# iammadab/zk

Hardware: AMD Instinct MI355X
Metric: field-ops/sec (MLE fold, 2^24 evals, BN254 Fr) + sumcheck prover wall-clock (higher is better)
Workload: dtype u256 (8 x u32 Montgomery limbs, integer)

## Files before the change

### zk_amd/csrc/gkr.hip

```cpp
#include <hip/hip_runtime.h>

#include <new>
#include <utility>
#include <vector>

#include "../../include/zk_amd.h"
#include "host_core.hpp"
#include "env.hpp"
#include "gkr_kernels.cuh"
#include "prover_state.hpp"


struct GkrLayer {
    uint32_t log_out, log_in;
    uint64_t n_gates, n_in;
    uint8_t *d_op;
    uint32_t *d_left, *d_right;
    uint32_t *d_lptr, *d_rptr;
    uint2 *d_lent, *d_rent;
    uint32_t *d_lheavy, *d_rheavy;
    uint32_t n_lheavy, n_rheavy;
    uint32_t *d_lptr_light, *d_rptr_light;
    uint2 *d_lent_light, *d_rent_light;
    uint8_t digest[112];
// ... 8 lines not shown
extern "C" int32_t zk_circuit_create(zk_ctx *c, zk_circuit **out) {
    if (!c || !out) return ZK_ERR_BAD_ARG;
    zk_circuit *z = new (std::nothrow) zk_circuit();
    if (!z) return ZK_ERR_ALLOC;
    z->ctx = c;
    *out = z;
    return ZK_OK;
}
extern "C" int32_t zk_circuit_free(zk_circuit *z) {
    if (!z) return ZK_OK;
    (void)use_device(z->ctx);
    delete z;
    return ZK_OK;
}
extern "C" int32_t zk_circuit_depth(const zk_circuit *z, uint64_t *out) {
    if (!z || !out) return ZK_ERR_BAD_ARG;
    *out = z->layers.size();
    return ZK_OK;
}
extern "C" int32_t zk_circuit_layer_dims(const zk_circuit *z, uint64_t layer, uint64_t *log_out, uint64_t *log_in) {
    if (!z || layer >= z->layers.size() || !log_out || !log_in) return ZK_ERR_BAD_ARG;
    *log_out = z->layers[layer].log_out;
    *log_in = z->layers[layer].log_in;
    return ZK_OK;
}
extern "C" int32_t zk_circuit_proof_elems(const zk_circuit *z, uint64_t *out) {
    if (!z || !out) return ZK_ERR_BAD_ARG;
    uint64_t n = 0;
    for (const auto &L : z->layers) n += 6ull * L.log_in + 2;
    *out = n;
    return ZK_OK;
}

static int32_t gkr_tree_reduce(zk_ctx *c, uint64_t *buf_a, uint64_t *buf_b, uint64_t n, uint64_t **root) {
    uint64_t *cur = buf_a, *nxt = buf_b;
    while (n > 1) {
        const uint64_t n_out = (n + 3) / 4;
        if (n_out <= 4096) k_tree_level_wave<<<(uint32_t)n_out, 64, 0, c->stream>>>(cur, n, nxt);
        else k_tree_level<<<grid_for(n_out), kBlock, 0, c->stream>>>(cur, n, n_out, nxt);
        HIPCHK(hipGetLastError());
        std::swap(cur, nxt);
        n = n_out;
    }
    *root = cur;
    return ZK_OK;
}
static int32_t gkr_table_digest_dev(zk_ctx *c, const zk_mle *t, uint64_t *d_out) {
    const uint64_t n = 1ull << t->n_vars, n_leaves = (n + 3) / 4;
    PoolScope ps(c);
    uint64_t *a = nullptr, *b = nullptr, *root = nullptr;
    ZKCHK(ps.get((size_t)n_leaves * 32, &a));
    ZKCHK(ps.get((size_t)((n_leaves + 3) / 4) * 32, &b));
    k_tree_leaves_table<<<grid_for(n_leaves), kBlock, 0, c->stream>>>(t->d, n, n_leaves, a, c->fi->P);
    HIPCHK(hipGetLastError());
    ZKCHK(gkr_tree_reduce(c, a, b, n_leaves, &root));
    HIPCHK(hipMemcpyAsync(d_out, root, 32, hipMemcpyDeviceToDevice, c->stream));
    return ZK_OK;
}
static int32_t gkr_bytes_digest(zk_ctx *c, const void *d_data, uint64_t nbytes, uint8_t out[32]) {
    const uint64_t n_leaves = nbytes ? (nbytes + 127) / 128 : 1;
    PoolScope ps(c);
    uint64_t *a = nullptr, *b = nullptr, *root = nullptr;
    ZKCHK(ps.get((size_t)n_leaves * 32, &a));
    ZKCHK(ps.get((size_t)((n_leaves + 3) / 4) * 32, &b));
    k_tree_leaves_bytes<<<grid_for(n_leaves), kBlock, 0, c->stream>>>((const uint8_t *)d_data, nbytes, n_leaves, a);
    HIPCHK(hipGetLastError());
    ZKCHK(gkr_tree_reduce(c, a, b, n_leaves, &root));
    HIPCHK(hipMemcpyAsync(out, root, 32, hipMemcpyDeviceToHost, c->stream));
    HIPCHK(hipStreamSynchronize(c->stream));
    return ZK_OK;
}
static void put_u64le(uint8_t *p, uint64_t v) {
    for (int i = 0; i < 8; ++i) p[i] = (uint8_t)(v >> (8 * i));
}
static void gkr_circuit_digest(const zk_circuit *z, uint8_t out[32]) {
    Sponge h;
    h.init();
    for (const auto &L : z->layers) h.update(L.digest, sizeof L.digest);
    h.finalize_reset(out);
}

template <typename T>
static int32_t gkr_upload(GkrLayer &L, T **dst, const T *src, size_t count) {
    if (L.n_blocks == (int)(sizeof L.blocks / sizeof L.blocks[0])) return ZK_ERR_ALLOC;
    RawBlock b;
    HIPCHK(hipMalloc(b.put(), (count ? count : 1) * sizeof(T)));
    if (count) HIPCHK(hipMemcpy(b.get(), src, count * sizeof(T), hipMemcpyHostToDevice));
    *dst = static_cast<T *>(b.get());
    L.blocks[L.n_blocks++] = std::move(b);
    return ZK_OK;
}
static int32_t gkr_upload_light(GkrLayer &L, const std::vector<uint32_t> &ptr, const std::vector<uint2> &ent, const std::vector<uint32_t> &heavy,
                                uint32_t *d_ptr, uint2 *d_ent, uint32_t **d_ptr_light, uint2 **d_ent_light) {
    if (heavy.empty()) {
        *d_ptr_light = d_ptr;
        *d_ent_light = d_ent;
        return ZK_OK;
    }
    const size_t rows = ptr.size() - 1;
    std::vector<uint32_t> lp(rows + 1, 0);
    std::vector<uint2> le;
// ... 72 lines not shown
    uint64_t *d_hi = nullptr, *d_lo = nullptr;
    ZKCHK(ps.get((size_t)32 << hi_bits, &d_hi));
    ZKCHK(ps.get((size_t)32 << lo_bits, &d_lo));
    {
        if (m <= 30) {
            const size_t lds = ((size_t)2 << ((lo_bits + 1) / 2)) * 32 + (size_t)2 * lo_bits * 32 + 64;
            k_eq_halves<<<2, kBlock, lds, c->stream>>>(d_point, (uint32_t)m, scale, d_hi, d_lo, P, d_scale);
        } else {
            k_eq_direct<<<grid_for(1ull << hi_bits), kBlock, 0, c->stream>>>(d_point, (uint32_t)hi_bits, scale, d_hi, P, d_scale);
            k_eq_direct<<<grid_for(1ull << lo_bits), kBlock, 0, c->stream>>>(d_point + 4 * hi_bits, (uint32_t)lo_bits, fe_one(P), d_lo, P);
        }
        if (accumulate)
            k_eq_outer<true><<<grid_for(1ull << m), kBlock, 0, c->stream>>>(d_hi, d_lo, (uint32_t)lo_bits, 1ull << m, d_out, P);
        else
            k_eq_outer<false><<<grid_for(1ull << m), kBlock, 0, c->stream>>>(d_hi, d_lo, (uint32_t)lo_bits, 1ull << m, d_out, P);
        HIPCHK(hipGetLastError());
    }
    return ZK_OK;
}
int32_t zk::eq_table_dev(zk_ctx *c, const uint64_t *d_point, uint64_t m, uint64_t *d_out) {
    return gkr_eq_table_dev(c, d_point, m, fe_one(c->fi->P), false, d_out);
}
static int32_t gkr_upload_point(zk_ctx *c, const uint64_t *point, uint64_t m, uint64_t *d_point) {
    if (m == 0) return ZK_OK;
    HIPCHK(hipMemcpyAsync(d_point, point, (size_t)m * 32, hipMemcpyHostToDevice, c->stream));
    HIPCHK(hipStreamSynchronize(c->stream));
    return ZK_OK;
}
struct EqHalves {
    PoolBlock buf;
    EqFactor f = {};
    void reset() { buf.reset(); }
};
static int32_t gkr_eq_halves(zk_ctx *c, const uint64_t *d_p1, const uint64_t *d_s1, const uint64_t *d_p2, const uint64_t *d_s2, uint64_t m,
                             EqHalves *out) {
    const FieldParams &P = c->fi->P;
    out->reset();
    out->f = {};
    if (m > 30) return ZK_ERR_UNSUPPORTED;
    const uint32_t lo_bits = eq_split_lo_bits(m), hi_bits = (uint32_t)m - lo_bits;
    const size_t hb = (size_t)32 << hi_bits, lb = (size_t)(kEqLoWords * 4) << lo_bits;
    ZKCHK(out->buf.alloc(c, (d_p2 ? 2 : 1) * (hb + lb)));
    uint64_t *hi1 = out->buf.as(), *lo1 = hi1 + hb / 8, *hi2 = d_p2 ? lo1 + lb / 8 : nullptr, *lo2 = d_p2 ? hi2 + hb / 8 : nullptr;
    const uint32_t bh = ((1u << hi_bits) + 1023) / 1024, bl = ((1u << lo_bits) + 1023) / 1024;
    const EqSplitJob j0 = {d_p1, d_s1, hi1, reinterpret_cast<uint32_t *>(lo1)}, j1 = {d_p2, d_s2, hi2, reinterpret_cast<uint32_t *>(lo2)};
    k_eq_split<<<(d_p2 ? 2 : 1) * (bh + bl), kBlock, 0, c->stream>>>(j0, j1, (uint32_t)m, lo_bits, bh, bl, P);
    HIPCHK(hipGetLastError());
    out->f = {hi1, hi2, reinterpret_cast<const uint32_t *>(lo1), reinterpret_cast<const uint32_t *>(lo2), lo_bits};
    return ZK_OK;
}
static int32_t gkr_eq_table(zk_ctx *c, const uint64_t *point, uint64_t m, const Fe *scale, bool accumulate, uint64_t *d_out) {
    PoolBlock d_point;
    ZKCHK(d_point.alloc(c, (size_t)(m ? m : 1) * 32));
    ZKCHK(gkr_upload_point(c, point, m, d_point.as()));
    return gkr_eq_table_dev(c, d_point.as(), m, scale ? *scale : fe_one(c->fi->P), accumulate, d_out);
}
extern "C" int32_t zk_eq_table(zk_ctx *c, const uint64_t *point, uint64_t n_vars, zk_mle **out) {
    if (!c || !out || (!point && n_vars)) return ZK_ERR_BAD_ARG;
    if (n_vars > kMaxVars) return ZK_ERR_UNSUPPORTED;
    ZKCHK(use_device(c));
    MleHolder t;
    ZKCHK(mle_alloc(c, n_vars, t.put()));
    ZKCHK(gkr_eq_table(c, point, n_vars, nullptr, false, t->d));
    *out = t.release();
    return ZK_OK;
}

static int32_t gkr_check_input(const zk_circuit *z, const zk_mle *input) {
    if (!z || !input) return ZK_ERR_BAD_ARG;
    if (z->layers.empty()) return ZK_ERR_BAD_ARG;
    if (input->ctx != z->ctx) return ZK_ERR_CONTEXT_MISMATCH;
    if (input->n_vars != z->layers.back().log_in) return ZK_ERR_ARITY_MISMATCH;
    return use_device(z->ctx);
}
struct GkrValues {
    std::vector<MleHolder> own;
    std::vector<zk_mle *> vals;
};
static int32_t gkr_forward(const zk_circuit *z, const zk_mle *input, GkrValues &v) {
    zk_ctx *c = z->ctx;
    const size_t d = z->layers.size();
    v.own.resize(d);
    v.vals.assign(d + 1, nullptr);
    v.vals[d] = const_cast<zk_mle *>(input);
    for (size_t i = d; i-- > 0;) {
        const GkrLayer &L = z->layers[i];
        ZKCHK(mle_alloc(c, L.log_out, v.own[i].put()));
        v.vals[i] = v.own[i].get();
        k_gkr_forward<<<grid_for(L.n_gates), kBlock, 0, c->stream>>>(L.d_op, L.d_left, L.d_right, v.vals[i + 1]->d, L.n_gates, v.vals[i]->d, c->fi->P);
        HIPCHK(hipGetLastError());
    }
    return ZK_OK;
}
extern "C" int32_t zk_gkr_evaluate(const zk_circuit *z, const zk_mle *input, zk_mle **out_outputs) {
    if (!out_outputs) return ZK_ERR_BAD_ARG;
    ZKCHK(gkr_check_input(z, input));
    GkrValues v;
    ZKCHK(gkr_forward(z, input, v));
    *out_outputs = v.own[0].release();
    return ZK_OK;
}

struct GkrClaim {
    std::vector<uint64_t> g1, g2;
    Fe alpha, beta, c;
    bool two;
};
static int32_t gkr_start(const zk_circuit *z, const zk_mle *input, const zk_mle *outputs, Sponge &sp, const uint8_t seed[32], GkrClaim &cl) {
    zk_ctx *c = z->ctx;
    const FieldParams &P = c->fi->P;
    const uint64_t log_out0 = z->layers[0].log_out;
    uint8_t cd[32], io[64];
    gkr_circuit_digest(z, cd);
    {
        PoolBlock d_dig;
        ZKCHK(d_dig.alloc(c, 64));
        ZKCHK(gkr_table_digest_dev(c, input, d_dig.as()));
        ZKCHK(gkr_table_digest_dev(c, outputs, d_dig.as() + 4));
        HIPCHK(hipMemcpyAsync(c->h_pinned, d_dig.p, 64, hipMemcpyDeviceToHost, c->stream));
        HIPCHK(hipStreamSynchronize(c->stream));
    }
    memcpy(io, c->h_pinned, 64);
    sp.init();
    sp.update(seed, 32);
    sp.update(cd, 32);
    sp.update(io, 64);
    cl.g1.assign(4 * log_out0, 0);
    for (uint64_t i = 0; i < log_out0; ++i) fe_to_u64limbs(squeeze_field_element(sp, P), cl.g1.data() + 4 * i);
    cl.g2.clear();
    cl.alpha = fe_one(P);
    cl.beta = fe_zero();
    cl.two = false;
    return ZK_OK;
}
static void gkr_next_claim(Sponge &sp, const FieldParams &P, const uint64_t *layer_proof, uint64_t log_in, const uint64_t *u,
                           const uint64_t *v, GkrClaim &cl) {
    cl.alpha = squeeze_field_element(sp, P);
    cl.beta = squeeze_field_element(sp, P);
    cl.two = true;
    cl.g1.assign(u, u + 4 * log_in);
    cl.g2.assign(v, v + 4 * log_in);
    const Fe wu = fe_from_u64limbs(layer_proof + 4 * (6 * log_in)), wv = fe_from_u64limbs(layer_proof + 4 * (6 * log_in + 1));
    cl.c = fe_add(fe_mul(cl.alpha, wu, P), fe_mul(cl.beta, wv, P), P);
}

extern "C" int32_t zk_gkr_prove(const zk_circuit *z, const zk_mle *input, const uint8_t seed[32], zk_mle **out_outputs,
                                uint64_t *out_proof) {
    if (!seed || !out_outputs || !out_proof) return ZK_ERR_BAD_ARG;
    ZKCHK(gkr_check_input(z, input));
    zk_ctx *c = z->ctx;
    const FieldParams &P = c->fi->P;
    const size_t d = z->layers.size();
    GkrValues v;
    PoolScope ps(c);
    DrainOnExit drain(c);
    ZKCHK(gkr_forward(z, input, v));
    const std::vector<zk_mle *> &vals = v.vals;
    uint64_t proof_elems = 0;
    (void)zk_circuit_proof_elems(z, &proof_elems);
    Sponge sp;
    GkrClaim cl;
    ZKCHK(gkr_start(z, input, vals[0], sp, seed, cl));
    constexpr size_t kPointBytes = 64 * 32;
    uint64_t *d_pt[4] = {nullptr, nullptr, nullptr, nullptr}, *d_fin = nullptr, *d_sc = nullptr, *d_proof = nullptr;
    WordSponge *d_sponge = nullptr;
    for (int i = 0; i < 4; ++i) ZKCHK(ps.get(kPointBytes, &d_pt[i]));
    ZKCHK(ps.get(kMaxFactors * 32, &d_fin));
    ZKCHK(ps.get(kGkrScalars * 32, &d_sc));
    ZKCHK(ps.get(sizeof(WordSponge), &d_sponge));
    ZKCHK(ps.get((size_t)proof_elems * 32, &d_proof));
    uint64_t *d_epart = nullptr;
    ZKCHK(ps.get(kEpartBlockBytes, &d_epart));
    uint64_t *d_g1 = d_pt[0], *d_g2 = d_pt[1], *d_u = d_pt[2], *d_v = d_pt[3];
    ZKCHK(gkr_upload_point(c, cl.g1.data(), z->layers[0].log_out, d_g1));
    ZKCHK(sponge_to_device(c, sp, d_sponge, d_epart));
    ZKCHK(evaluate_device(c, vals[0], cl.g1.data(), d_sc + 4 * kGkrScClaim));
    k_gkr_chain_start<<<1, 64, 0, c->stream>>>(d_sponge, d_sc, P);
    HIPCHK(hipGetLastError());
    bool two = false;
    uint64_t *proof = d_proof;
    for (size_t i = 0; i < d; ++i) {
        const GkrLayer &L = z->layers[i];
        const uint64_t s = L.log_in;
        MleHolder H, B, H2, C2;
        ZKCHK(mle_alloc(c, s, H.put()));
        ZKCHK(mle_alloc(c, s, B.put()));
        ZKCHK(mle_alloc(c, s, H2.put()));
        ZKCHK(mle_alloc(c, s, C2.put()));
        EqHalves hE, hU;
        ZKCHK(gkr_eq_halves(c, d_g1, two ? d_sc + 4 * kGkrScAlpha : nullptr, two ? d_g2 : nullptr, two ? d_sc + 4 * kGkrScBeta : nullptr, L.log_out, &hE));
        k_gkr_phase<1><<<gkr_phase_grid(L.n_in), kBlock, 0, c->stream>>>(L.d_lptr_light, L.d_lent_light, hE.f, vals[i + 1]->d, EqFactor{}, nullptr, L.n_in,
                                                                         H->d, B->d, P);
        if (L.n_lheavy) k_gkr_phase1_heavy<<<L.n_lheavy, kBlock, 0, c->stream>>>(L.d_lheavy, L.d_lptr, L.d_lent, hE.f, vals[i + 1]->d, H->d, B->d, P);
        HIPCHK(hipGetLastError());
        TermSpec ts = {2, {2, 1, 0, 0}};
        zk_mle *f1[3] = {vals[i + 1], H.get(), B.get()};
        const DeviceChain ch1 = {d_sponge, proof, d_u, d_fin, d_epart};
        ZKCHK(prove_core(c, f1, 3, ts, 2, nullptr, 0, 0, nullptr, nullptr, nullptr, nullptr, nullptr, nullptr, &ch1));
        k_gkr_chain_mid<<<1, 64, 0, c->stream>>>(d_sponge, d_fin, proof + 4 * (6 * s), d_sc, P);
        HIPCHK(hipGetLastError());
        ZKCHK(gkr_eq_halves(c, d_u, nullptr, d_u, d_fin, s, &hU));
        k_gkr_phase<2><<<gkr_phase_grid(L.n_in), kBlock, 0, c->stream>>>(L.d_rptr_light, L.d_rent_light, hE.f, nullptr, hU.f, d_fin, L.n_in, H2->d, C2->d, P);
        if (L.n_rheavy) k_gkr_phase2_heavy<<<L.n_rheavy, kBlock, 0, c->stream>>>(L.d_rheavy, L.d_rptr, L.d_rent, hE.f, hU.f, d_fin, H2->d, C2->d, P);
        HIPCHK(hipGetLastError());
        hE.reset();
        hU.reset();
        zk_mle *f2[3] = {vals[i + 1], H2.get(), C2.get()};
        const DeviceChain ch2 = {d_sponge, proof + 4 * (3 * s), d_v, d_fin, d_epart};
        ZKCHK(prove_core(c, f2, 3, ts, 2, nullptr, 0, 0, nullptr, nullptr, nullptr, nullptr, nullptr, nullptr, &ch2));
        k_gkr_chain_end<<<1, 64, 0, c->stream>>>(d_sponge, d_fin, proof + 4 * (6 * s), proof + 4 * (6 * s + 1), d_sc, P);
        HIPCHK(hipGetLastError());
        proof += 4 * (6 * s + 2);
        std::swap(d_g1, d_u);
        std::swap(d_g2, d_v);
        two = true;
    }
    HIPCHK(hipMemcpyAsync(out_proof, d_proof, (size_t)proof_elems * 32, hipMemcpyDeviceToHost, c->stream));
    ZKCHK(drain.wait());
    *out_outputs = v.own[0].release();
    return ZK_OK;
}

struct GkrLayerCheck {
    Fe sub2, wu, wv;
};
extern "C" int32_t zk_gkr_verify(const zk_circuit *z, const zk_mle *input, const zk_mle *outputs, const uint8_t seed[32],
                                 const uint64_t *proof_in) {
    if (!seed || !outputs || !proof_in) return ZK_ERR_BAD_ARG;
    ZKCHK(gkr_check_input(z, input));
    zk_ctx *c = z->ctx;
    if (outputs->ctx != c) return ZK_ERR_CONTEXT_MISMATCH;
    if (outputs->n_vars != z->layers[0].log_out) return ZK_ERR_ARITY_MISMATCH;
    const FieldParams &P = c->fi->P;
    const size_t d = z->layers.size();
// ... 121 lines not shown
```

### zk_amd/csrc/gkr_kernels.cuh

```cuda
#pragma once
#include "common.cuh"
#include "transcript.cuh"

namespace zk {

__global__ __launch_bounds__(kBlock) void k_eq_direct(const uint64_t *__restrict__ point, uint32_t nv, Fe scale,
                                                      uint64_t *__restrict__ out, FieldParams P, const uint64_t *__restrict__ d_scale = nullptr) {
    if (d_scale) scale = fe_load(d_scale, 0);
    const uint64_t n = 1ull << nv, stride = (uint64_t)gridDim.x * kBlock;
    Fe one;
#pragma unroll
    for (int i = 0; i < 8; ++i) one.v[i] = P.r1[i];
    for (uint64_t j = (uint64_t)blockIdx.x * kBlock + threadIdx.x; j < n; j += stride) {
        Fe acc = scale;
        for (uint32_t w = 0; w < nv; ++w) {
            const Fe g = fe_load(point, w);
            const bool bit = (j >> (nv - 1 - w)) & 1;
            acc = fe_mul(acc, bit ? g : fe_sub(one, g, P), P);
        }
        fe_store(out, j, acc);
    }
}
template <bool ACCUMULATE>
__global__ __launch_bounds__(kBlock) void k_eq_outer(const uint64_t *__restrict__ hi, const uint64_t *__restrict__ lo,
// ... 52 lines not shown
        const uint32_t j = in_a ? e : e - na, cnt = in_a ? a : b, off = in_a ? 0 : a;
        Fe acc = (in_a && is_hi) ? scale : one;
        for (uint32_t w = 0; w < cnt; ++w) acc = fe_mul(acc, fe_load(pt, 2 * (off + w) + ((j >> (cnt - 1 - w)) & 1)), P);
        fe_store(in_a ? qa : qb, j, acc);
    }
    __syncthreads();
    uint64_t *dst = is_hi ? d_hi : d_lo;
    for (uint32_t i = threadIdx.x; i < (1u << nv); i += kBlock) fe_store(dst, i, fe_mul(fe_load(qa, i >> b), fe_load(qb, i & (nb - 1)), P));
}

struct EqFactor {
    const uint64_t *hi, *hi2;
    const uint32_t *lo, *lo2;
    uint32_t lo_bits;
};
ZK_D Fe eq_factor_at(const EqFactor &f, uint32_t i, const FieldParams &P) {
    const uint32_t h = i >> f.lo_bits, l = i & ((1u << f.lo_bits) - 1);
    const Fe a = fe_load(f.hi, h);
    const Mul29 c = load_eq_lo(f.lo + (size_t)l * kEqLoWords);
    if (!f.hi2) return fe_mul29(a, c, P);
    return fe_dot2_29(a, c, fe_load(f.hi2, h), load_eq_lo(f.lo2 + (size_t)l * kEqLoWords), P);
}

ZK_D Fe eq_u_at(const EqFactor &f, uint32_t i, bool scaled, const FieldParams &P) {
    const uint32_t h = i >> f.lo_bits, l = i & ((1u << f.lo_bits) - 1);
    return fe_mul29(fe_load(scaled ? f.hi2 : f.hi, h), load_eq_lo(f.lo + (size_t)l * kEqLoWords), P);
}
struct EqSplitJob {
    const uint64_t *point, *scale;
    uint64_t *hi;
    uint32_t *lo;
};
static inline uint32_t eq_split_lo_bits(uint64_t m) { return (uint32_t)(m <= 7 ? m : (m > 23 ? m - 16 : 7)); }
__global__ __launch_bounds__(kBlock) void k_eq_split(EqSplitJob j0, EqSplitJob j1, uint32_t m, uint32_t lo_bits, uint32_t bh, uint32_t bl,
                                                     FieldParams P) {
    __shared__ uint64_t qa[256 * 4], qb[256 * 4], pt[2 * 16 * 4];
    const uint32_t per = bh + bl, slot = blockIdx.x % per;
    const EqSplitJob job = blockIdx.x / per ? j1 : j0;
    const bool is_hi = slot < bh;
    const uint32_t slice = is_hi ? slot : slot - bh;
    const uint32_t nv = is_hi ? m - lo_bits : lo_bits, first = is_hi ? 0 : m - lo_bits;
    const uint32_t a = nv / 2, b = nv - a, na = 1u << a, nb = 1u << b;
    Fe one;
#pragma unroll
    for (int i = 0; i < 8; ++i) one.v[i] = P.r1[i];
    if (threadIdx.x < nv) {
        const Fe g = fe_load(job.point, first + threadIdx.x);
        fe_store(pt, 2 * threadIdx.x, fe_sub(one, g, P));
        fe_store(pt, 2 * threadIdx.x + 1, g);
    }
    __syncthreads();
    const Fe scale = (is_hi && job.scale) ? fe_load(job.scale, 0) : one;
    for (uint32_t e = threadIdx.x; e < na + nb; e += kBlock) {
        const bool in_a = e < na;
        const uint32_t j = in_a ? e : e - na, cnt = in_a ? a : b, off = in_a ? 0 : a;
        Fe acc = in_a ? scale : one;
        for (uint32_t w = 0; w < cnt; ++w) acc = fe_mul(acc, fe_load(pt, 2 * (off + w) + ((j >> (cnt - 1 - w)) & 1)), P);
        fe_store(in_a ? qa : qb, j, acc);
    }
    __syncthreads();
    const uint32_t end = (slice + 1) * 1024 < (1u << nv) ? (slice + 1) * 1024 : (1u << nv);
    for (uint32_t i = slice * 1024 + threadIdx.x; i < end; i += kBlock) {
        const Fe v = fe_mul(fe_load(qa, i >> b), fe_load(qb, i & (nb - 1)), P);
        if (is_hi) fe_store(job.hi, i, v);
        else store_eq_lo(job.lo + (size_t)i * kEqLoWords, mul29_prepare(v, P));
    }
}

__global__ __launch_bounds__(kBlock) void k_gkr_forward(const uint8_t *__restrict__ op, const uint32_t *__restrict__ left,
                                                        const uint32_t *__restrict__ right, const uint64_t *__restrict__ W,
                                                        uint64_t n_gates, uint64_t *__restrict__ out, FieldParams P) {
    const uint64_t stride = (uint64_t)gridDim.x * kBlock;
    for (uint64_t z = (uint64_t)blockIdx.x * kBlock + threadIdx.x; z < n_gates; z += stride) {
        const Fe a = fe_load(W, left[z]), b = fe_load(W, right[z]);
        fe_store(out, z, op[z] ? fe_mul(a, b, P) : fe_add(a, b, P));
    }
}

constexpr uint32_t kGkrHeavyRow = 256;
ZK_D void gkr_block_sum2(Fe (&sum)[2], const FieldParams &P) {
    __shared__ uint32_t red2[kBlock / 64][2][8];
    const int lane = threadIdx.x & 63, wave = threadIdx.x >> 6;
#pragma unroll
    for (int t = 0; t < 2; ++t) {
        sum[t] = fe_wave_sum(sum[t], P);
        if (lane == 0) {
#pragma unroll
            for (int i = 0; i < 8; ++i) red2[wave][t][i] = sum[t].v[i];
        }
    }
    __syncthreads();
    if (threadIdx.x == 0) {
#pragma unroll
        for (int t = 0; t < 2; ++t) {
            Fe acc = fe_zero();
            for (int w = 0; w < kBlock / 64; ++w) {
                Fe o;
#pragma unroll
                for (int i = 0; i < 8; ++i) o.v[i] = red2[w][t][i];
                acc = fe_add(acc, o, P);
            }
            sum[t] = acc;
        }
    }
}
__global__ __launch_bounds__(kBlock) void k_gkr_phase1_heavy(const uint32_t *__restrict__ heavy, const uint32_t *__restrict__ lptr,
                                                             const uint2 *__restrict__ lent, EqFactor E,
                                                             const uint64_t *__restrict__ W, uint64_t *__restrict__ H,
                                                             uint64_t *__restrict__ B1, FieldParams P) {
// ... 129 lines not shown
    const uint64_t stride = (uint64_t)gridDim.x * kBlock, first = (uint64_t)blockIdx.x * kBlock + threadIdx.x;
    if (first >= n) return;
    Fe cur = scale, b = base;
    for (uint64_t e = first; e; e >>= 1) {
        if (e & 1) cur = fe_mul(cur, b, P);
        b = fe_mul(b, b, P);
    }
    for (uint64_t j = first; j < n; j += stride) {
        fe_store(t, j, fe_mul(fe_load(t, j), cur, P));
        cur = fe_mul(cur, step, P);
    }
}
__global__ __launch_bounds__(kBlock) void k_dft_across(const uint64_t *__restrict__ in, uint64_t *__restrict__ out, uint32_t W,
                                                       uint64_t L, const uint64_t *__restrict__ pw, FieldParams P) {
    const uint64_t stride = (uint64_t)gridDim.x * kBlock;
    for (uint64_t j = (uint64_t)blockIdx.x * kBlock + threadIdx.x; j < L; j += stride) {
        for (uint32_t k = 0; k < W; ++k) {
            Fe acc = fe_load(in, j);
            for (uint32_t r = 1; r < W; ++r) acc = fe_add(acc, fe_mul(fe_load(in, (uint64_t)r * L + j), fe_load(pw, (r * k) & (W - 1)), P), P);
            fe_store(out, (uint64_t)k * L + j, acc);
        }
    }
}

constexpr int kGkrScClaim = 0, kGkrScAlpha = 1, kGkrScBeta = 2, kGkrScSum2 = 3, kGkrScalars = 4;
__global__ __launch_bounds__(64) void k_gkr_chain_start(WordSponge *__restrict__ gsp, const uint64_t *__restrict__ sc, FieldParams P) {
    __shared__ Fe buf[2];
    const LaneKeccak L = lane_keccak_init();
    LaneSponge sp = lane_sponge_load(gsp, L);
    if (L.lane == 0) buf[0] = fe_load(sc, kGkrScClaim);
    lane_absorb_elems(sp, L, buf, 1, P);
    lane_sponge_store(gsp, sp, L);
}
__global__ __launch_bounds__(64) void k_gkr_chain_mid(WordSponge *__restrict__ gsp, const uint64_t *__restrict__ fin, uint64_t *__restrict__ proof_wu,
                                                       uint64_t *__restrict__ sc, FieldParams P) {
    __shared__ Fe buf[2];
    const LaneKeccak L = lane_keccak_init();
    LaneSponge sp = lane_sponge_load(gsp, L);
    if (L.lane == 0) {
        const Fe wu = fe_load(fin, 0), hu = fe_load(fin, 1), bu = fe_load(fin, 2);
        const Fe s2 = fe_add(fe_mul(wu, hu, P), bu, P);
        buf[0] = wu;
        buf[1] = s2;
        fe_store(proof_wu, 0, wu);
        fe_store(sc, kGkrScSum2, s2);
    }
    lane_absorb_elems(sp, L, buf, 2, P);
    lane_sponge_store(gsp, sp, L);
}
__global__ __launch_bounds__(64) void k_gkr_chain_end(WordSponge *__restrict__ gsp, const uint64_t *__restrict__ fin, const uint64_t *__restrict__ proof_wu,
                                                       uint64_t *__restrict__ proof_wv, uint64_t *__restrict__ sc, FieldParams P) {
    __shared__ Fe buf[2];
    const LaneKeccak L = lane_keccak_init();
    LaneSponge sp = lane_sponge_load(gsp, L);
    const Fe wu = fe_load(proof_wu, 0), wv = fe_load(fin, 0);
    if (L.lane == 0) {
        buf[0] = wv;
        fe_store(proof_wv, 0, wv);
    }
    lane_absorb_elems(sp, L, buf, 1, P);
    Mul29 t29;
    const Fe alpha = lane_squeeze(sp, L, P, t29), beta = lane_squeeze(sp, L, P, t29);
    const Fe claim = fe_add(fe_mul(alpha, wu, P), fe_mul(beta, wv, P), P);
    if (L.lane == 0) {
        buf[1] = claim;
        fe_store(sc, kGkrScAlpha, alpha);
        fe_store(sc, kGkrScBeta, beta);
        fe_store(sc, kGkrScClaim, claim);
    }
    lane_absorb_elems(sp, L, buf + 1, 1, P);
    lane_sponge_store(gsp, sp, L);
}

ZK_D void tree_keccak_finish(uint64_t (&s)[25], uint32_t len_bytes, uint64_t *__restrict__ out) {
    s[len_bytes >> 3] ^= 0x01ull << (8 * (len_bytes & 7));
    s[16] ^= 0x8000000000000000ull;
    keccak_f1600(s);
#pragma unroll
    for (int i = 0; i < 4; ++i) out[i] = s[i];
}
__global__ __launch_bounds__(kBlock) void k_tree_leaves_table(const uint64_t *__restrict__ table, uint64_t n_elems, uint64_t n_leaves,
                                                              uint64_t *__restrict__ out, FieldParams P) {
    const uint64_t stride = (uint64_t)gridDim.x * kBlock;
    for (uint64_t i = (uint64_t)blockIdx.x * kBlock + threadIdx.x; i < n_leaves; i += stride) {
        uint64_t s[25];
#pragma unroll
        for (int k = 0; k < 25; ++k) s[k] = 0;
        uint32_t len = 0;
#pragma unroll
        for (int e = 0; e < 4; ++e) {
            if (4 * i + e < n_elems) {
                const Fe c = fe_to_canonical(fe_load(table, 4 * i + e), P);
#pragma unroll
                for (int w = 0; w < 4; ++w)
                    s[4 * e + w] = WordSponge::bswap64((uint64_t)c.v[2 * (3 - w)] | ((uint64_t)c.v[2 * (3 - w) + 1] << 32));
                len += 32;
            }
        }
        tree_keccak_finish(s, len, out + 4 * i);
    }
}
__global__ __launch_bounds__(kBlock) void k_tree_leaves_bytes(const uint8_t *__restrict__ data, uint64_t nbytes, uint64_t n_leaves,
                                                              uint64_t *__restrict__ out) {
    const uint64_t stride = (uint64_t)gridDim.x * kBlock;
    for (uint64_t i = (uint64_t)blockIdx.x * kBlock + threadIdx.x; i < n_leaves; i += stride) {
        uint64_t s[25];
#pragma unroll
        for (int k = 0; k < 25; ++k) s[k] = 0;
        const uint64_t base = 128 * i;
        const uint32_t len = (uint32_t)(nbytes - base < 128 ? nbytes - base : 128);
#pragma unroll
        for (int w = 0; w < 16; ++w) {
            uint64_t x = 0;
            for (int b = 0; b < 8; ++b)
                if ((uint32_t)(8 * w + b) < len) x |= (uint64_t)data[base + 8 * w + b] << (8 * b);
            s[w] = x;
        }
        tree_keccak_finish(s, len, out + 4 * i);
    }
}
__global__ __launch_bounds__(kBlock) void k_tree_level(const uint64_t *__restrict__ in, uint64_t n_in, uint64_t n_out, uint64_t *__restrict__ out) {
    const uint64_t stride = (uint64_t)gridDim.x * kBlock;
    for (uint64_t j = (uint64_t)blockIdx.x * kBlock + threadIdx.x; j < n_out; j += stride) {
        uint64_t s[25];
#pragma unroll
        for (int k = 0; k < 25; ++k) s[k] = 0;
        uint32_t len = 0;
#pragma unroll
        for (int c = 0; c < 4; ++c) {
            if (4 * j + c < n_in) {
#pragma unroll
                for (int w = 0; w < 4; ++w) s[4 * c + w] = in[4 * (4 * j + c) + w];
                len += 32;
            }
        }
        tree_keccak_finish(s, len, out + 4 * j);
    }
}
__global__ __launch_bounds__(64) void k_tree_level_wave(const uint64_t *__restrict__ in, uint64_t n_in, uint64_t *__restrict__ out) {
    const uint64_t j = blockIdx.x;
    const LaneKeccak L = lane_keccak_init();
    const uint64_t rem = n_in - 4 * j;
    const uint32_t nwords = 4 * (uint32_t)(rem < 4 ? rem : 4);
    uint64_t a = 0;
    if (L.index >= 0 && (uint32_t)L.index < nwords) a = in[16 * j + (uint32_t)L.index];
    if ((uint32_t)L.index == nwords) a ^= 0x01ull;
    if (L.index == 16) a ^= 0x8000000000000000ull;
    a = lane_keccak_f1600(a, L);
    if (L.index >= 0 && L.index < 4) out[4 * j + (uint32_t)L.index] = a;
}

}
```

Before: 195.1 billion.

## Fuse Merkle tree levels in LDS and piggyback hashing on GKR kernels

Replaces the per-level Keccak Merkle reduction (one launch per 4:1 level) with a block-local kernel that computes leaves and several levels inside shared memory. Two independent tree chains (input and output digests) now run in one 2D launch. The input-table digest is spread across the GKR forward-pass launches as extra blocks, and the chain-mid sponge step is merged into the eq-split launch. The aim is to cut kernel launches and global round trips, at the cost of more shared-memory use and more complex kernels.

```diff
diff --git a/zk_amd/csrc/gkr.hip b/zk_amd/csrc/gkr.hip
--- a/zk_amd/csrc/gkr.hip
+++ b/zk_amd/csrc/gkr.hip
@@ -64,41 +64,69 @@
     return ZK_OK;
 }
 
-static int32_t gkr_tree_reduce(zk_ctx *c, uint64_t *buf_a, uint64_t *buf_b, uint64_t n, uint64_t **root) {
-    uint64_t *cur = buf_a, *nxt = buf_b;
-    while (n > 1) {
-        const uint64_t n_out = (n + 3) / 4;
-        if (n_out <= 4096) k_tree_level_wave<<<(uint32_t)n_out, 64, 0, c->stream>>>(cur, n, nxt);
-        else k_tree_level<<<grid_for(n_out), kBlock, 0, c->stream>>>(cur, n, n_out, nxt);
+struct TreeChain {
+    TreeJob job = {};
+    uint64_t *buf[2] = {nullptr, nullptr}, *dst = nullptr;
+    int flip = 0;
+    bool done = true;
+};
+static int32_t tree_chain_begin(PoolScope &ps, TreeChain &t, uint32_t kind, const void *src, uint64_t n_src, uint64_t n_leaves, uint64_t *dst,
+                                uint32_t first_unit = kTreeUnit) {
+    t = TreeChain();
+    t.job = {src, n_src, n_leaves, nullptr, kind};
+    t.dst = dst;
+    t.done = false;
+    const uint64_t n1 = (n_leaves + first_unit - 1) / first_unit, n2 = (n1 + kTreeUnit - 1) / kTreeUnit;
+    if (n1 > 1) ZKCHK(ps.get((size_t)n1 * 32, &t.buf[0]));
+    if (n2 > 1) ZKCHK(ps.get((size_t)n2 * 32, &t.buf[1]));
+    return ZK_OK;
+}
+static uint64_t tree_chain_stage(TreeChain &t, uint32_t unit) {
+    const uint64_t units = (t.job.n + unit - 1) / unit;
+    t.job.out = units == 1 ? t.dst : t.buf[t.flip];
+    return units;
+}
+static void tree_chain_advance(TreeChain &t, uint64_t units) {
+    if (units == 1) {
+        t.done = true;
+        return;
+    }
+    t.job = {t.job.out, 0, units, nullptr, kTreeDigests};
+    t.flip ^= 1;
+}
+static int32_t tree_chains_run(zk_ctx *c, TreeChain *a, TreeChain *b) {
+    TreeChain *all[2] = {a, b};
+    for (;;) {
+        TreeChain *who[2];
+        TreeJob j[2] = {};
+        uint64_t units[2] = {0, 0};
+        uint32_t nj = 0;
+        for (TreeChain *t : all) {
+            if (!t || t->done) continue;
+            units[nj] = tree_chain_stage(*t, kTreeUnit);
+            j[nj] = t->job;
+            who[nj++] = t;
+        }
+        if (!nj) return ZK_OK;
+        const uint64_t gx = units[0] > units[1] ? units[0] : units[1];
+        if (gx > 0x7FFFFFFFull) return ZK_ERR_UNSUPPORTED;
+        k_tree_stage<<<dim3((uint32_t)gx, nj), kBlock, 0, c->stream>>>(j[0], j[1], c->fi->P);
         HIPCHK(hipGetLastError());
-        std::swap(cur, nxt);
-        n = n_out;
-    }
-    *root = cur;
-    return ZK_OK;
-}
-static int32_t gkr_table_digest_dev(zk_ctx *c, const zk_mle *t, uint64_t *d_out) {
-    const uint64_t n = 1ull << t->n_vars, n_leaves = (n + 3) / 4;
+        for (uint32_t i = 0; i < nj; ++i) tree_chain_advance(*who[i], units[i]);
+    }
+}
+static int32_t tree_chain_begin_table(PoolScope &ps, TreeChain &t, const zk_mle *tab, uint64_t *dst, uint32_t first_unit = kTreeUnit) {
+    const uint64_t n = 1ull << tab->n_vars;
+    return tree_chain_begin(ps, t, kTreeTable, tab->d, n, (n + 3) / 4, dst, first_unit);
+}
+static int32_t gkr_bytes_digest(zk_ctx *c, const void *d_data, uint64_t nbytes, uint8_t out[32]) {
     PoolScope ps(c);
-    uint64_t *a = nullptr, *b = nullptr, *root = nullptr;
-    ZKCHK(ps.get((size_t)n_leaves * 32, &a));
-    ZKCHK(ps.get((size_t)((n_leaves + 3) / 4) * 32, &b));
-    k_tree_leaves_table<<<grid_for(n_leaves), kBlock, 0, c->stream>>>(t->d, n, n_leaves, a, c->fi->P);
-    HIPCHK(hipGetLastError());
-    ZKCHK(gkr_tree_reduce(c, a, b, n_leaves, &root));
-    HIPCHK(hipMemcpyAsync(d_out, root, 32, hipMemcpyDeviceToDevice, c->stream));
-    return ZK_OK;
-}
-static int32_t gkr_bytes_digest(zk_ctx *c, const void *d_data, uint64_t nbytes, uint8_t out[32]) {
-    const uint64_t n_leaves = nbytes ? (nbytes + 127) / 128 : 1;
-    PoolScope ps(c);
-    uint64_t *a = nullptr, *b = nullptr, *root = nullptr;
-    ZKCHK(ps.get((size_t)n_leaves * 32, &a));
-    ZKCHK(ps.get((size_t)((n_leaves + 3) / 4) * 32, &b));
-    k_tree_leaves_bytes<<<grid_for(n_leaves), kBlock, 0, c->stream>>>((const uint8_t *)d_data, nbytes, n_leaves, a);
-    HIPCHK(hipGetLastError());
-    ZKCHK(gkr_tree_reduce(c, a, b, n_leaves, &root));
-    HIPCHK(hipMemcpyAsync(out, root, 32, hipMemcpyDeviceToHost, c->stream));
+    uint64_t *d_root = nullptr;
+    ZKCHK(ps.get(32, &d_root));
+    TreeChain t;
+    ZKCHK(tree_chain_begin(ps, t, kTreeBytes, d_data, nbytes, nbytes ? (nbytes + 127) / 128 : 1, d_root));
+    ZKCHK(tree_chains_run(c, &t, nullptr));
+    HIPCHK(hipMemcpyAsync(out, d_root, 32, hipMemcpyDeviceToHost, c->stream));
     HIPCHK(hipStreamSynchronize(c->stream));
     return ZK_OK;
 }
@@ -237,8 +265,13 @@
     EqFactor f = {};
     void reset() { buf.reset(); }
 };
+struct GkrMidStep {
+    WordSponge *sponge;
+    const uint64_t *fin;
+    uint64_t *proof_wu, *sc;
+};
 static int32_t gkr_eq_halves(zk_ctx *c, const uint64_t *d_p1, const uint64_t *d_s1, const uint64_t *d_p2, const uint64_t *d_s2, uint64_t m,
-                             EqHalves *out) {
+                             EqHalves *out, const GkrMidStep *mid = nullptr) {
     const FieldParams &P = c->fi->P;
     out->reset();
     out->f = {};
@@ -249,7 +282,9 @@
     uint64_t *hi1 = out->buf.as(), *lo1 = hi1 + hb / 8, *hi2 = d_p2 ? lo1 + lb / 8 : nullptr, *lo2 = d_p2 ? hi2 + hb / 8 : nullptr;
     const uint32_t bh = ((1u << hi_bits) + 1023) / 1024, bl = ((1u << lo_bits) + 1023) / 1024;
     const EqSplitJob j0 = {d_p1, d_s1, hi1, reinterpret_cast<uint32_t *>(lo1)}, j1 = {d_p2, d_s2, hi2, reinterpret_cast<uint32_t *>(lo2)};
-    k_eq_split<<<(d_p2 ? 2 : 1) * (bh + bl), kBlock, 0, c->stream>>>(j0, j1, (uint32_t)m, lo_bits, bh, bl, P);
+    const uint32_t g = (d_p2 ? 2 : 1) * (bh + bl);
+    if (mid) k_gkr_chain_mid_eq<<<1 + g, kBlock, 0, c->stream>>>(mid->sponge, mid->fin, mid->proof_wu, mid->sc, j0, j1, (uint32_t)m, lo_bits, bh, bl, P);
+    else k_eq_split<<<g, kBlock, 0, c->stream>>>(j0, j1, (uint32_t)m, lo_bits, bh, bl, P);
     HIPCHK(hipGetLastError());
     out->f = {hi1, hi2, reinterpret_cast<const uint32_t *>(lo1), reinterpret_cast<const uint32_t *>(lo2), lo_bits};
     return ZK_OK;
@@ -282,19 +317,27 @@
     std::vector<MleHolder> own;
     std::vector<zk_mle *> vals;
 };
-static int32_t gkr_forward(const zk_circuit *z, const zk_mle *input, GkrValues &v) {
+static int32_t gkr_forward(const zk_circuit *z, const zk_mle *input, GkrValues &v, TreeChain *rider = nullptr) {
     zk_ctx *c = z->ctx;
     const size_t d = z->layers.size();
     v.own.resize(d);
     v.vals.assign(d + 1, nullptr);
     v.vals[d] = const_cast<zk_mle *>(input);
-    for (size_t i = d; i-- > 0;) {
+    const uint64_t units = rider ? tree_chain_stage(*rider, kTreeRiderUnit) : 0;
+    for (size_t i = d, k = 0; i-- > 0; ++k) {
         const GkrLayer &L = z->layers[i];
         ZKCHK(mle_alloc(c, L.log_out, v.own[i].put()));
         v.vals[i] = v.own[i].get();
-        k_gkr_forward<<<grid_for(L.n_gates), kBlock, 0, c->stream>>>(L.d_op, L.d_left, L.d_right, v.vals[i + 1]->d, L.n_gates, v.vals[i]->d, c->fi->P);
+        TreeRider r = {};
+        if (rider) {
+            const uint64_t first = units * k / d;
+            r = {rider->job, (uint32_t)first, (uint32_t)(units * (k + 1) / d - first)};
+        }
+        k_gkr_forward<<<r.n_units + grid_for(L.n_gates), kBlock, 0, c->stream>>>(L.d_op, L.d_left, L.d_right, v.vals[i + 1]->d, L.n_gates, v.vals[i]->d,
+                                                                               c->fi->P, r);
         HIPCHK(hipGetLastError());
     }
+    if (rider) tree_chain_advance(*rider, units);
     return ZK_OK;
 }
 extern "C" int32_t zk_gkr_evaluate(const zk_circuit *z, const zk_mle *input, zk_mle **out_outputs) {
@@ -311,18 +354,24 @@
     Fe alpha, beta, c;
     bool two;
 };
-static int32_t gkr_start(const zk_circuit *z, const zk_mle *input, const zk_mle *outputs, Sponge &sp, const uint8_t seed[32], GkrClaim &cl) {
+static int32_t gkr_start(const zk_circuit *z, const zk_mle *input, const zk_mle *outputs, Sponge &sp, const uint8_t seed[32], GkrClaim &cl,
+                         TreeChain *in_chain = nullptr, uint64_t *d_dig = nullptr) {
     zk_ctx *c = z->ctx;
     const FieldParams &P = c->fi->P;
     const uint64_t log_out0 = z->layers[0].log_out;
     uint8_t cd[32], io[64];
     gkr_circuit_digest(z, cd);
     {
-        PoolBlock d_dig;
-        ZKCHK(d_dig.alloc(c, 64));
-        ZKCHK(gkr_table_digest_dev(c, input, d_dig.as()));
-        ZKCHK(gkr_table_digest_dev(c, outputs, d_dig.as() + 4));
-        HIPCHK(hipMemcpyAsync(c->h_pinned, d_dig.p, 64, hipMemcpyDeviceToHost, c->stream));
+        PoolScope ps(c);
+        TreeChain t_in, t_out;
+        if (!in_chain) {
+            ZKCHK(ps.get(64, &d_dig));
+            ZKCHK(tree_chain_begin_table(ps, t_in, input, d_dig));
+            in_chain = &t_in;
+        }
+        ZKCHK(tree_chain_begin_table(ps, t_out, outputs, d_dig + 4));
+        ZKCHK(tree_chains_run(c, &t_out, in_chain));
+        HIPCHK(hipMemcpyAsync(c->h_pinned, d_dig, 64, hipMemcpyDeviceToHost, c->stream));
         HIPCHK(hipStreamSynchronize(c->stream));
     }
     memcpy(io, c->h_pinned, 64);
@@ -359,13 +408,17 @@
     GkrValues v;
     PoolScope ps(c);
     DrainOnExit drain(c);
-    ZKCHK(gkr_forward(z, input, v));
+    uint64_t *d_dig = nullptr;
+    TreeChain t_in;
+    ZKCHK(ps.get(64, &d_dig));
+    ZKCHK(tree_chain_begin_table(ps, t_in, input, d_dig, kTreeRiderUnit));
+    ZKCHK(gkr_forward(z, input, v, &t_in));
     const std::vector<zk_mle *> &vals = v.vals;
     uint64_t proof_elems = 0;
     (void)zk_circuit_proof_elems(z, &proof_elems);
     Sponge sp;
     GkrClaim cl;
-    ZKCHK(gkr_start(z, input, vals[0], sp, seed, cl));
+    ZKCHK(gkr_start(z, input, vals[0], sp, seed, cl, &t_in, d_dig));
     constexpr size_t kPointBytes = 64 * 32;
     uint64_t *d_pt[4] = {nullptr, nullptr, nullptr, nullptr}, *d_fin = nullptr, *d_sc = nullptr, *d_proof = nullptr;
     WordSponge *d_sponge = nullptr;
@@ -402,9 +455,8 @@
         zk_mle *f1[3] = {vals[i + 1], H.get(), B.get()};
         const DeviceChain ch1 = {d_sponge, proof, d_u, d_fin, d_epart};
         ZKCHK(prove_core(c, f1, 3, ts, 2, nullptr, 0, 0, nullptr, nullptr, nullptr, nullptr, nullptr, nullptr, &ch1));
-        k_gkr_chain_mid<<<1, 64, 0, c->stream>>>(d_sponge, d_fin, proof + 4 * (6 * s), d_sc, P);
-        HIPCHK(hipGetLastError());
-        ZKCHK(gkr_eq_halves(c, d_u, nullptr, d_u, d_fin, s, &hU));
+        const GkrMidStep mid = {d_sponge, d_fin, proof + 4 * (6 * s), d_sc};
+        ZKCHK(gkr_eq_halves(c, d_u, nullptr, d_u, d_fin, s, &hU, &mid));
         k_gkr_phase<2><<<gkr_phase_grid(L.n_in), kBlock, 0, c->stream>>>(L.d_rptr_light, L.d_rent_light, hE.f, nullptr, hU.f, d_fin, L.n_in, H2->d, C2->d, P);
         if (L.n_rheavy) k_gkr_phase2_heavy<<<L.n_rheavy, kBlock, 0, c->stream>>>(L.d_rheavy, L.d_rptr, L.d_rent, hE.f, hU.f, d_fin, H2->d, C2->d, P);
         HIPCHK(hipGetLastError());
diff --git a/zk_amd/csrc/gkr_kernels.cuh b/zk_amd/csrc/gkr_kernels.cuh
--- a/zk_amd/csrc/gkr_kernels.cuh
+++ b/zk_amd/csrc/gkr_kernels.cuh
@@ -108,11 +108,11 @@
     uint32_t *lo;
 };
 static inline uint32_t eq_split_lo_bits(uint64_t m) { return (uint32_t)(m <= 7 ? m : (m > 23 ? m - 16 : 7)); }
-__global__ __launch_bounds__(kBlock) void k_eq_split(EqSplitJob j0, EqSplitJob j1, uint32_t m, uint32_t lo_bits, uint32_t bh, uint32_t bl,
-                                                     FieldParams P) {
+ZK_D void eq_split_block(const EqSplitJob &j0, const EqSplitJob &j1, uint32_t m, uint32_t lo_bits, uint32_t bh, uint32_t bl, const FieldParams &P,
+                         uint32_t block) {
     __shared__ uint64_t qa[256 * 4], qb[256 * 4], pt[2 * 16 * 4];
-    const uint32_t per = bh + bl, slot = blockIdx.x % per;
-    const EqSplitJob job = blockIdx.x / per ? j1 : j0;
+    const uint32_t per = bh + bl, slot = block % per;
+    const EqSplitJob job = block / per ? j1 : j0;
     const bool is_hi = slot < bh;
     const uint32_t slice = is_hi ? slot : slot - bh;
     const uint32_t nv = is_hi ? m - lo_bits : lo_bits, first = is_hi ? 0 : m - lo_bits;
@@ -142,15 +142,9 @@
         else store_eq_lo(job.lo + (size_t)i * kEqLoWords, mul29_prepare(v, P));
     }
 }
-
-__global__ __launch_bounds__(kBlock) void k_gkr_forward(const uint8_t *__restrict__ op, const uint32_t *__restrict__ left,
-                                                        const uint32_t *__restrict__ right, const uint64_t *__restrict__ W,
-                                                        uint64_t n_gates, uint64_t *__restrict__ out, FieldParams P) {
-    const uint64_t stride = (uint64_t)gridDim.x * kBlock;
-    for (uint64_t z = (uint64_t)blockIdx.x * kBlock + threadIdx.x; z < n_gates; z += stride) {
-        const Fe a = fe_load(W, left[z]), b = fe_load(W, right[z]);
-        fe_store(out, z, op[z] ? fe_mul(a, b, P) : fe_add(a, b, P));
-    }
+__global__ __launch_bounds__(kBlock) void k_eq_split(EqSplitJob j0, EqSplitJob j1, uint32_t m, uint32_t lo_bits, uint32_t bh, uint32_t bl,
+                                                     FieldParams P) {
+    eq_split_block(j0, j1, m, lo_bits, bh, bl, P, blockIdx.x);
 }
 
 constexpr uint32_t kGkrHeavyRow = 256;
@@ -346,8 +340,14 @@
     lane_absorb_elems(sp, L, buf, 1, P);
     lane_sponge_store(gsp, sp, L);
 }
-__global__ __launch_bounds__(64) void k_gkr_chain_mid(WordSponge *__restrict__ gsp, const uint64_t *__restrict__ fin, uint64_t *__restrict__ proof_wu,
-                                                       uint64_t *__restrict__ sc, FieldParams P) {
+__global__ __launch_bounds__(kBlock) void k_gkr_chain_mid_eq(WordSponge *__restrict__ gsp, const uint64_t *__restrict__ fin, uint64_t *__restrict__ proof_wu,
+                                                             uint64_t *__restrict__ sc, EqSplitJob j0, EqSplitJob j1, uint32_t m, uint32_t lo_bits,
+                                                             uint32_t bh, uint32_t bl, FieldParams P) {
+    if (blockIdx.x) {
+        eq_split_block(j0, j1, m, lo_bits, bh, bl, P, blockIdx.x - 1);
+        return;
+    }
+    if (threadIdx.x >= 64) return;
     __shared__ Fe buf[2];
     const LaneKeccak L = lane_keccak_init();
     LaneSponge sp = lane_sponge_load(gsp, L);
@@ -386,82 +386,143 @@
     lane_sponge_store(gsp, sp, L);
 }
 
-ZK_D void tree_keccak_finish(uint64_t (&s)[25], uint32_t len_bytes, uint64_t *__restrict__ out) {
-    s[len_bytes >> 3] ^= 0x01ull << (8 * (len_bytes & 7));
+ZK_D void tree_keccak_finish(uint64_t (&s)[25], uint32_t len_bytes, uint64_t *out) {
+    const uint64_t pad = 0x01ull << (8 * (len_bytes & 7));
+#pragma unroll
+    for (uint32_t k = 0; k <= 16; ++k) s[k] ^= k == (len_bytes >> 3) ? pad : 0ull;
     s[16] ^= 0x8000000000000000ull;
     keccak_f1600(s);
 #pragma unroll
     for (int i = 0; i < 4; ++i) out[i] = s[i];
 }
-__global__ __launch_bounds__(kBlock) void k_tree_leaves_table(const uint64_t *__restrict__ table, uint64_t n_elems, uint64_t n_leaves,
-                                                              uint64_t *__restrict__ out, FieldParams P) {
-    const uint64_t stride = (uint64_t)gridDim.x * kBlock;
-    for (uint64_t i = (uint64_t)blockIdx.x * kBlock + threadIdx.x; i < n_leaves; i += stride) {
-        uint64_t s[25];
-#pragma unroll
-        for (int k = 0; k < 25; ++k) s[k] = 0;
-        uint32_t len = 0;
-#pragma unroll
-        for (int e = 0; e < 4; ++e) {
-            if (4 * i + e < n_elems) {
-                const Fe c = fe_to_canonical(fe_load(table, 4 * i + e), P);
-#pragma unroll
-                for (int w = 0; w < 4; ++w)
-                    s[4 * e + w] = WordSponge::bswap64((uint64_t)c.v[2 * (3 - w)] | ((uint64_t)c.v[2 * (3 - w) + 1] << 32));
-                len += 32;
+ZK_D void tree_leaf_table(const uint64_t *__restrict__ table, uint64_t n_elems, uint64_t i, const FieldParams &P, uint64_t *out) {
+    uint64_t s[25];
+#pragma unroll
+    for (int k = 0; k < 25; ++k) s[k] = 0;
+    uint32_t len = 0;
+#pragma unroll
+    for (int e = 0; e < 4; ++e) {
+        if (4 * i + e < n_elems) {
+            const Fe c = fe_to_canonical(fe_load(table, 4 * i + e), P);
+#pragma unroll
+            for (int w = 0; w < 4; ++w)
+                s[4 * e + w] = WordSponge::bswap64((uint64_t)c.v[2 * (3 - w)] | ((uint64_t)c.v[2 * (3 - w) + 1] << 32));
+            len += 32;
+        }
+    }
+    tree_keccak_finish(s, len, out);
+}
+ZK_D void tree_leaf_bytes(const uint8_t *__restrict__ data, uint64_t nbytes, uint64_t i, uint64_t *out) {
+    uint64_t s[25];
+#pragma unroll
+    for (int k = 0; k < 25; ++k) s[k] = 0;
+    const uint64_t base = 128 * i;
+    const uint32_t len = (uint32_t)(nbytes - base < 128 ? nbytes - base : 128);
+#pragma unroll
+    for (int w = 0; w < 16; ++w) {
+        uint64_t x = 0;
+        for (int b = 0; b < 8; ++b)
+            if ((uint32_t)(8 * w + b) < len) x |= (uint64_t)data[base + 8 * w + b] << (8 * b);
+        s[w] = x;
+    }
+    tree_keccak_finish(s, len, out);
+}
+constexpr uint32_t kTreeTable = 0, kTreeBytes = 1, kTreeDigests = 2;
+constexpr uint32_t kTreeWaveNodes = 16;
+constexpr uint32_t kTreeUnit = 1024;
+constexpr uint32_t kTreeRiderUnit = 64;
+struct TreeJob {
+    const void *src;
+    uint64_t n_src;
+    uint64_t n;
+    uint64_t *out;
+    uint32_t kind;
+};
+template <uint32_t U>
+ZK_D void tree_unit(const TreeJob &j, uint64_t unit, const FieldParams &P, uint64_t *lds) {
+    const uint64_t first = unit * U;
+    uint32_t cnt = (uint32_t)(j.n - first < U ? j.n - first : U);
+    uint64_t *cur = lds, *nxt = lds + (size_t)U * 4;
+    for (uint32_t t = threadIdx.x; t < cnt; t += kBlock) {
+        uint64_t d[4];
+        if (j.kind == kTreeTable) {
+            tree_leaf_table(static_cast<const uint64_t *>(j.src), j.n_src, first + t, P, d);
+        } else if (j.kind == kTreeBytes) {
+            tree_leaf_bytes(static_cast<const uint8_t *>(j.src), j.n_src, first + t, d);
+        } else {
+#pragma unroll
+            for (int w = 0; w < 4; ++w) d[w] = static_cast<const uint64_t *>(j.src)[4 * (first + t) + w];
+        }
+#pragma unroll
+        for (int w = 0; w < 4; ++w) cur[4 * t + w] = d[w];
+    }
+    __syncthreads();
+    constexpr int kLevels = U == 1024 ? 5 : (U == 256 ? 4 : 3);
+    static_assert(U == 64 || U == 256 || U == 1024, "U = 4^levels, and a level of U / 4 nodes has a thread each");
+    uint64_t n_glob = j.n;
+    for (int l = 0; l < kLevels && n_glob > 1; ++l, n_glob = (n_glob + 3) / 4) {
+        const uint32_t n_out = (cnt + 3) / 4;
+        if (n_out > kTreeWaveNodes) {
+            if (threadIdx.x < n_out) {
+                uint64_t s[25];
+#pragma unroll
+                for (int k = 0; k < 25; ++k) s[k] = 0;
+                uint32_t len = 0;
+#pragma unroll
+                for (int c = 0; c < 4; ++c) {
+                    if (4 * threadIdx.x + c < cnt) {
+#pragma unroll
+                        for (int w = 0; w < 4; ++w) s[4 * c + w] = cur[4 * (4 * threadIdx.x + c) + w];
+                        len += 32;
+                    }
+                }
+                tree_keccak_finish(s, len, nxt + 4 * threadIdx.x);
             }
-        }
-        tree_keccak_finish(s, len, out + 4 * i);
-    }
-}
-__global__ __launch_bounds__(kBlock) void k_tree_leaves_bytes(const uint8_t *__restrict__ data, uint64_t nbytes, uint64_t n_leaves,
-                                                              uint64_t *__restrict__ out) {
-    const uint64_t stride = (uint64_t)gridDim.x * kBlock;
-    for (uint64_t i = (uint64_t)blockIdx.x * kBlock + threadIdx.x; i < n_leaves; i += stride) {
-        uint64_t s[25];
-#pragma unroll
-        for (int k = 0; k < 25; ++k) s[k] = 0;
-        const uint64_t base = 128 * i;
-        const uint32_t len = (uint32_t)(nbytes - base < 128 ? nbytes - base : 128);
-#pragma unroll
-        for (int w = 0; w < 16; ++w) {
-            uint64_t x = 0;
-            for (int b = 0; b < 8; ++b)
-                if ((uint32_t)(8 * w + b) < len) x |= (uint64_t)data[base + 8 * w + b] << (8 * b);
-            s[w] = x;
-        }
-        tree_keccak_finish(s, len, out + 4 * i);
-    }
-}
-__global__ __launch_bounds__(kBlock) void k_tree_level(const uint64_t *__restrict__ in, uint64_t n_in, uint64_t n_out, uint64_t *__restrict__ out) {
-    const uint64_t stride = (uint64_t)gridDim.x * kBlock;
-    for (uint64_t j = (uint64_t)blockIdx.x * kBlock + threadIdx.x; j < n_out; j += stride) {
-        uint64_t s[25];
-#pragma unroll
-        for (int k = 0; k < 25; ++k) s[k] = 0;
-        uint32_t len = 0;
-#pragma unroll
-        for (int c = 0; c < 4; ++c) {
-            if (4 * j + c < n_in) {
-#pragma unroll
-                for (int w = 0; w < 4; ++w) s[4 * c + w] = in[4 * (4 * j + c) + w];
-                len += 32;
+        } else {
+            const LaneKeccak L = lane_keccak_init();
+            for (uint32_t k = threadIdx.x >> 6; k < n_out; k += kBlock / 64) {
+                const uint32_t rem = cnt - 4 * k, nwords = 4 * (rem < 4 ? rem : 4);
+                uint64_t a = 0;
+                if (L.index >= 0 && (uint32_t)L.index < nwords) a = cur[16 * k + (uint32_t)L.index];
+                if ((uint32_t)L.index == nwords) a ^= 0x01ull;
+                if (L.index == 16) a ^= 0x8000000000000000ull;
+                a = lane_keccak_f1600(a, L);
+                if (L.index >= 0 && L.index < 4) nxt[4 * k + (uint32_t)L.index] = a;
             }
         }
-        tree_keccak_finish(s, len, out + 4 * j);
-    }
-}
-__global__ __launch_bounds__(64) void k_tree_level_wave(const uint64_t *__restrict__ in, uint64_t n_in, uint64_t *__restrict__ out) {
-    const uint64_t j = blockIdx.x;
-    const LaneKeccak L = lane_keccak_init();
-    const uint64_t rem = n_in - 4 * j;
-    const uint32_t nwords = 4 * (uint32_t)(rem < 4 ? rem : 4);
-    uint64_t a = 0;
-    if (L.index >= 0 && (uint32_t)L.index < nwords) a = in[16 * j + (uint32_t)L.index];
-    if ((uint32_t)L.index == nwords) a ^= 0x01ull;
-    if (L.index == 16) a ^= 0x8000000000000000ull;
-    a = lane_keccak_f1600(a, L);
-    if (L.index >= 0 && L.index < 4) out[4 * j + (uint32_t)L.index] = a;
-}
-
-}
+        __syncthreads();
+        uint64_t *t = cur;
+        cur = nxt;
+        nxt = t;
+        cnt = n_out;
+    }
+    if (threadIdx.x < 4) j.out[4 * unit + threadIdx.x] = cur[threadIdx.x];
+}
+__global__ __launch_bounds__(kBlock) void k_tree_stage(TreeJob j0, TreeJob j1, FieldParams P) {
+    constexpr uint32_t U = kTreeUnit;
+    __shared__ uint64_t lds[U * 4 + U];
+    const TreeJob &j = blockIdx.y ? j1 : j0;
+    if ((uint64_t)blockIdx.x * U >= j.n) return;
+    tree_unit<U>(j, blockIdx.x, P, lds);
+}
+
+struct TreeRider {
+    TreeJob job;
+    uint32_t first_unit, n_units;
+};
+__global__ __launch_bounds__(kBlock) void k_gkr_forward(const uint8_t *__restrict__ op, const uint32_t *__restrict__ left,
+                                                        const uint32_t *__restrict__ right, const uint64_t *__restrict__ W,
+                                                        uint64_t n_gates, uint64_t *__restrict__ out, FieldParams P, TreeRider rider) {
+    if (blockIdx.x < rider.n_units) {
+        __shared__ uint64_t lds[kTreeRiderUnit * 4 + kTreeRiderUnit];
+        tree_unit<kTreeRiderUnit>(rider.job, rider.first_unit + blockIdx.x, P, lds);
+        return;
+    }
+    const uint64_t stride = (uint64_t)(gridDim.x - rider.n_units) * kBlock;
+    for (uint64_t z = (uint64_t)(blockIdx.x - rider.n_units) * kBlock + threadIdx.x; z < n_gates; z += stride) {
+        const Fe a = fe_load(W, left[z]), b = fe_load(W, right[z]);
+        fe_store(out, z, op[z] ? fe_mul(a, b, P) : fe_add(a, b, P));
+    }
+}
+
+}
```

Result: no change. 195.7 billion (median of 6 runs) (+0.3%).
